# nikolovjovan/exblas

Measured on AMD Instinct MI355X. Metric: ExSUM fp64 Gelem/s at n=2^28 (bit-exact vs CPU superaccumulator/MPFR), higher is better.
Workload: dtype f64; 1 GPU; ExSUM n=2^28 fp64 ill_cond(c=1e+32), fpe=8 early_exit=True, 1xMI355X, inputs resident in HBM, steps rotate over 4 distinct vectors; n_total=268435456, fpe=8, early_exit=True, parallelism=single

## Files before the change

exblas_amd/csrc/blas1.hip:

```cpp
#include "superacc.hip.h"
#include "fpe.hip.h"
#include "exblas_internal.h"
#include <hip/hip_ext.h>

namespace exb {

constexpr int BLOCK = 256;
constexpr int WAVES = BLOCK / 64;
constexpr int U = 4;

template <int N, bool EE, int COPIES, int CNT, int ZM = 0>
__device__ __forceinline__ void fpe_absorb(double (&a)[N > 0 ? N : 1], double (&x)[CNT], int from,
                                           long long *col, unsigned &flags)
{
    LdsSink<COPIES> sink{col, flags};
    fpe_absorb_sink<N, EE, CNT, LdsSink<COPIES>, ZM>(a, x, from, sink);
}

template <int N, int COPIES>
__device__ __forceinline__ void fpe_flush(double (&a)[N > 0 ? N : 1], long long *col, unsigned &flags)
{
    LdsSink<COPIES> sink{col, flags};
    fpe_flush_sink<N>(a, sink);
}

template <int COPIES>
__device__ __forceinline__ void block_epilogue(long long *s_acc, unsigned flags, long long *gacc,
                                               unsigned *gflags, int ngroups)
{
    __shared__ unsigned s_flags;
    if (threadIdx.x == 0) s_flags = 0;
    __syncthreads();
    if (flags) atomicOr(&s_flags, flags);
    long long *g = gacc + (size_t)(blockIdx.x % ngroups) * NL;
    for (int l = threadIdx.x; l < NL; l += BLOCK) {
        long long sum = 0;
#pragma unroll
        for (int w = 0; w < WAVES; ++w)
#pragma unroll
            for (int c = 0; c < COPIES; ++c) sum += s_acc[(w * NL + l) * COPIES + c];
        if (sum != 0) atomicAdd((unsigned long long *)&g[l], (unsigned long long)sum);
    }
    __syncthreads();
    if (threadIdx.x == 0 && s_flags) atomicOr(gflags, s_flags);
}

template <int N, bool EE, int COPIES>
__global__ void __launch_bounds__(BLOCK) k_exsum(const double *__restrict__ a, long long n,
                                                 long long *__restrict__ gacc,
                                                 unsigned *__restrict__ gflags, int ngroups)
{
    __shared__ long long s_acc[WAVES * NL * COPIES];
    auto zero_lds = [&]() {
        for (int i = threadIdx.x; i < WAVES * NL * COPIES; i += BLOCK) s_acc[i] = 0;
        __syncthreads();
    };
    const int wave = threadIdx.x >> 6, lane = threadIdx.x & 63;
    long long *col = s_acc + wave * NL * COPIES + (lane & (COPIES - 1));
    unsigned flags = 0;
    double fpe[N > 0 ? N : 1];
#pragma unroll
    for (int i = 0; i < (N > 0 ? N : 1); ++i) fpe[i] = 0.0;

    const long long head = (((uintptr_t)a & 8u) && n > 0) ? 1 : 0;
    const d2_t *v = (const d2_t *)(a + head);
    const long long nv = (n - head) >> 1;
    constexpr long long TILE = (long long)BLOCK * U;
    const long long ntiles = nv / TILE;
    LdsSink<COPIES> sinkm{col, flags};
    Bypass bypass;

    long long t = blockIdx.x;
    if (t < ntiles) {
        d2_t r0[U], r1[U];
        auto fill = [&](long long tile, d2_t (&r)[U]) {
            const d2_t *p = v + (tile < ntiles ? tile : ntiles - 1) * TILE + threadIdx.x;
#pragma unroll
            for (int u = 0; u < U; ++u) r[u] = ld2(p + u * BLOCK);
        };
        auto absorb = [&](d2_t (&r)[U]) {
            double x[2 * U];
#pragma unroll
            for (int u = 0; u < U; ++u) {
                x[2 * u] = r[u].x;
                x[2 * u + 1] = r[u].y;
            }
            fpe_absorb_adaptive<N, EE, 2 * U, LdsSink<COPIES>>(fpe, x, sinkm, bypass);
        };
        fill(t, r0);
        zero_lds();
        for (;;) {
            fill(t + gridDim.x, r1);
            absorb(r0);
            t += gridDim.x;
            if (t >= ntiles) break;
            fill(t + gridDim.x, r0);
            absorb(r1);
            t += gridDim.x;
            if (t >= ntiles) break;
        }
    } else {
        zero_lds();
    }
    for (long long i = ntiles * TILE + (long long)blockIdx.x * BLOCK + threadIdx.x; i < nv;
         i += (long long)gridDim.x * BLOCK) {
        d2_t r = v[i];
        double x[2] = {r.x, r.y};
        fpe_absorb<N, false, COPIES, 2>(fpe, x, 0, col, flags);
    }
    if (blockIdx.x == 0 && threadIdx.x == 0) {
        if (head) lds_add<COPIES>(col, a[0], flags);
        if ((n - head) & 1) lds_add<COPIES>(col, a[n - 1], flags);
    }
    fpe_flush<N, COPIES>(fpe, col, flags);
    block_epilogue<COPIES>(s_acc, flags, gacc, gflags, ngroups);
}

template <int N, bool EE, int COPIES>
__global__ void __launch_bounds__(BLOCK) k_exsum_strided(const double *__restrict__ a, long long n,
                                                         long long inca, long long *__restrict__ gacc,
                                                         unsigned *__restrict__ gflags, int ngroups)
{
    __shared__ long long s_acc[WAVES * NL * COPIES];
    for (int i = threadIdx.x; i < WAVES * NL * COPIES; i += BLOCK) s_acc[i] = 0;
    __syncthreads();
    const int wave = threadIdx.x >> 6, lane = threadIdx.x & 63;
    long long *col = s_acc + wave * NL * COPIES + (lane & (COPIES - 1));
    unsigned flags = 0;
    double fpe[N > 0 ? N : 1];
#pragma unroll
    for (int i = 0; i < (N > 0 ? N : 1); ++i) fpe[i] = 0.0;
    const long long T = (long long)gridDim.x * BLOCK;
    for (long long i = (long long)blockIdx.x * BLOCK + threadIdx.x; i < n; i += 4 * T) {
        double x[4];
#pragma unroll
        for (int u = 0; u < 4; ++u) x[u] = i + u * T < n ? a[(i + u * T) * inca] : 0.0;
        fpe_absorb<N, false, COPIES, 4>(fpe, x, 0, col, flags);
    }
    fpe_flush<N, COPIES>(fpe, col, flags);
    block_epilogue<COPIES>(s_acc, flags, gacc, gflags, ngroups);
}

template <int N, bool EE, int COPIES, int ZM>
__global__ void __launch_bounds__(BLOCK) k_exdot(const double *__restrict__ a, const double *__restrict__ b,
                                                 long long n, long long *__restrict__ gacc,
                                                 unsigned *__restrict__ gflags, int ngroups)
{
    __shared__ long long s_acc[WAVES * NL * COPIES];
    auto zero_lds = [&]() {
        for (int i = threadIdx.x; i < WAVES * NL * COPIES; i += BLOCK) s_acc[i] = 0;
        __syncthreads();
    };
    const int wave = threadIdx.x >> 6, lane = threadIdx.x & 63;
    long long *col = s_acc + wave * NL * COPIES + (lane & (COPIES - 1));
    unsigned flags = 0;
    LdsSink<COPIES> sink{col, flags};
    long long *const lo_acc = low_acc_of(gflags), *const hi_acc = high_acc_of(gflags);
    double fpe[N > 0 ? N : 1];
#pragma unroll
    for (int i = 0; i < (N > 0 ? N : 1); ++i) fpe[i] = 0.0;

    const d2_t *va = (const d2_t *)a, *vb = (const d2_t *)b;
    const long long nv = n >> 1;
    Bypass bypass;
    constexpr long long TILE = (long long)BLOCK * U;
    const long long ntiles = nv / TILE;
    long long t = blockIdx.x;
    d2_t ra[U], rb[U];
    if (t < ntiles) {
        const long long base = t * TILE + threadIdx.x;
#pragma unroll
        for (int u = 0; u < U; ++u) {
            ra[u] = ld2(va + base + u * BLOCK);
            rb[u] = ld2(vb + base + u * BLOCK);
        }
    }
    zero_lds();
    if (t < ntiles) {
        d2_t rc[U], rd[U];
        auto fill = [&](long long tile, d2_t (&pa)[U], d2_t (&pb)[U]) {
            const long long base = (tile < ntiles ? tile : ntiles - 1) * TILE + threadIdx.x;
#pragma unroll
            for (int u = 0; u < U; ++u) {
                pa[u] = ld2(va + base + u * BLOCK);
                pb[u] = ld2(vb + base + u * BLOCK);
            }
        };
        auto absorb = [&](d2_t (&pa)[U], d2_t (&pb)[U]) {
            double x[2 * U], e[2 * U];
#pragma unroll
            for (int u = 0; u < U; ++u) {
                x[2 * u] = two_prod(pa[u].x, pb[u].x, e[2 * u]);
                x[2 * u + 1] = two_prod(pa[u].y, pb[u].y, e[2 * u + 1]);
            }
            if (!prod_range_divert<2 * U>(fpe[0], x, e, sink, lo_acc, hi_acc, [&](int j) { return j & 1 ? pa[j >> 1].y : pa[j >> 1].x; },
                                              [&](int j) { return j & 1 ? pb[j >> 1].y : pb[j >> 1].x; }))
                fpe_absorb_prod_adaptive<N, EE, 2 * U, LdsSink<COPIES>, ZM, false>(fpe, x, e, sink, bypass);
        };
        for (;;) {
            fill(t + gridDim.x, rc, rd);
            absorb(ra, rb);
            t += gridDim.x;
            if (t >= ntiles) break;
            fill(t + gridDim.x, ra, rb);
            absorb(rc, rd);
            t += gridDim.x;
            if (t >= ntiles) break;
        }
    }
    for (long long i = ntiles * TILE + (long long)blockIdx.x * BLOCK + threadIdx.x; i < nv;
         i += (long long)gridDim.x * BLOCK) {
        d2_t ra = va[i], rb = vb[i];
        double x[2], e[2];
        x[0] = two_prod(ra.x, rb.x, e[0]);
        x[1] = two_prod(ra.y, rb.y, e[1]);
        if (!prod_range_divert<2>(fpe[0], x, e, sink, lo_acc, hi_acc, [&](int j) { return j ? ra.y : ra.x; }, [&](int j) { return j ? rb.y : rb.x; }))
            fpe_absorb_prod<N, false, 2, LdsSink<COPIES>, 0, false>(fpe, x, e, sink);
    }
    if (blockIdx.x == 0 && threadIdx.x == 0 && (n & 1)) {
        double x1[1], e1[1];
        x1[0] = two_prod(a[n - 1], b[n - 1], e1[0]);
        if (!prod_range_divert<1>(fpe[0], x1, e1, sink, lo_acc, hi_acc, [&](int) { return a[n - 1]; }, [&](int) { return b[n - 1]; }))
            sink_product(sink, x1[0], e1[0]);
    }
    fpe_flush<N, COPIES>(fpe, col, flags);
    block_epilogue<COPIES>(s_acc, flags, gacc, gflags, ngroups);
}

template <int N, bool EE, int COPIES>
__global__ void __launch_bounds__(BLOCK) k_exdot_strided(const double *__restrict__ a, long long inca,
                                                         const double *__restrict__ b, long long incb,
                                                         long long n, long long *__restrict__ gacc,
                                                         unsigned *__restrict__ gflags, int ngroups)
{
    __shared__ long long s_acc[WAVES * NL * COPIES];
    for (int i = threadIdx.x; i < WAVES * NL * COPIES; i += BLOCK) s_acc[i] = 0;
    __syncthreads();
    const int wave = threadIdx.x >> 6, lane = threadIdx.x & 63;
    long long *col = s_acc + wave * NL * COPIES + (lane & (COPIES - 1));
    unsigned flags = 0;
    LdsSink<COPIES> sink{col, flags};
    long long *const lo_acc = low_acc_of(gflags), *const hi_acc = high_acc_of(gflags);
    double fpe[N > 0 ? N : 1];
#pragma unroll
    for (int i = 0; i < (N > 0 ? N : 1); ++i) fpe[i] = 0.0;
    const long long T = (long long)gridDim.x * BLOCK;
    for (long long i = (long long)blockIdx.x * BLOCK + threadIdx.x; i < n; i += 4 * T) {
        double va[4], vb[4], x[4], e[4];
#pragma unroll
        for (int u = 0; u < 4; ++u) {
            const bool in = i + u * T < n;
            va[u] = in ? a[(i + u * T) * inca] : 0.0;
            vb[u] = in ? b[(i + u * T) * incb] : 0.0;
        }
#pragma unroll
        for (int u = 0; u < 4; ++u) x[u] = two_prod(va[u], vb[u], e[u]);
        if (!prod_range_divert<4>(fpe[0], x, e, sink, lo_acc, hi_acc, [&](int j) { return va[j]; }, [&](int j) { return vb[j]; }))
            fpe_absorb_prod<N, false, 4, LdsSink<COPIES>, 0, false>(fpe, x, e, sink);
    }
    fpe_flush<N, COPIES>(fpe, col, flags);
    block_epilogue<COPIES>(s_acc, flags, gacc, gflags, ngroups);
}

__global__ void __launch_bounds__(64) k_finalize(long long *sets, int nsets, int set_stride, unsigned *gflags,
                                                 unsigned flags_or, int zero_sets, long long *out,
                                                 const long long *ext_in, long long *ext_out)
{
    const int lane = threadIdx.x;
    unsigned flags = flags_or;
    if (gflags) flags |= *gflags;
    if (set_stride >= SET_WORDS) {
        for (int g = 0; g < nsets; ++g)
        {
            for (int k = 0; k < 3; ++k)
                if (sets[(size_t)g * set_stride + NL + k] != 0) flags |= (1u << k);
            const long long pw = sets[(size_t)g * set_stride + NL + 3];
            if (pw & 0xffff) flags |= FLAG_PUNDER;
            if (pw >> 16) flags |= FLAG_POVER;
        }
    }
    long long lo0 = 0, hi0 = 0, lo1 = 0, hi1 = 0;
    for (int g0 = 0; g0 < nsets; g0 += 16) {
        long long t0[16], t1[16];
#pragma unroll
        for (int k = 0; k < 16; ++k) {
            const bool ok = g0 + k < nsets;
            const long long *p = sets + (size_t)(ok ? g0 + k : 0) * set_stride;
            t0[k] = ok ? __builtin_nontemporal_load(p + lane) : 0;
            t1[k] = (ok && lane < NL - 64) ? __builtin_nontemporal_load(p + 64 + lane) : 0;
        }
#pragma unroll
        for (int k = 0; k < 16; ++k) {
            lo0 += t0[k] & 0xffffffffll;
            hi0 += t0[k] >> 32;
            if (lane == NL - 65) {
                lo1 += t1[k];
            } else {
                lo1 += t1[k] & 0xffffffffll;
                hi1 += t1[k] >> 32;
            }
        }
    }
    long long in0 = __shfl_up(hi0, 1), in1 = __shfl_up(hi1, 1);
    const long long h63 = __shfl(hi0, 63);
    if (lane == 0) { in0 = 0; in1 = h63; }
    long long v0 = lo0 + in0, v1 = (lane < NL - 64) ? lo1 + in1 : 0;
    if (zero_sets) {
        for (int i = lane; i < nsets * set_stride; i += 64) sets[i] = 0;
        if (lane == 0 && gflags) *gflags = 0;
    }
    __shared__ long long s_v[NL], s_lo[NL], s_hi[NL], s_c[NL + EXT_SHIFT_DIGITS];
    __shared__ unsigned long long s_ex;
    __shared__ int s_over;
    bool low_folded = false;
    const bool have_low = (flags & FLAG_PUNDER) && (ext_in || gflags);
    const bool have_high = (flags & FLAG_POVER) && (ext_in || gflags);
    if (ext_out) {
        if (!have_low) {
            ext_out[lane] = 0;
            if (lane < SET_WORDS - 64) ext_out[64 + lane] = 0;
        }
        if (!have_high) {
            ext_out[SET_WORDS + lane] = 0;
            if (lane < SET_WORDS - 64) ext_out[SET_WORDS + 64 + lane] = 0;
        }
    }
    if (have_low || have_high) {
        const long long *lsrc = ext_in ? ext_in : low_acc_of(gflags);
        const long long *hsrc = ext_in ? ext_in + SET_WORDS : high_acc_of(gflags);
        s_lo[lane] = have_low ? lsrc[lane] : 0;
        s_hi[lane] = have_high ? hsrc[lane] : 0;
        s_v[lane] = v0;
        if (lane < NL - 64) {
            s_lo[64 + lane] = have_low ? lsrc[64 + lane] : 0;
            s_hi[64 + lane] = have_high ? hsrc[64 + lane] : 0;
            s_v[64 + lane] = v1;
        }
        if (!ext_in && zero_sets) {
            long long *lo = low_acc_of(gflags), *hi = high_acc_of(gflags);
            if (have_low) {
                lo[lane] = 0;
                if (lane < NL - 64) lo[64 + lane] = 0;
            }
            if (have_high) {
                hi[lane] = 0;
                if (lane < NL - 64) hi[64 + lane] = 0;
            }
        }
        __syncthreads();
        if (lane == 0) {
            s_over = 0;
            if (have_low) normalize_digits(s_lo);
            if (have_high) normalize_digits(s_hi);
            if (!ext_out) {
                if (have_high) s_over = fold_high_digits(s_v, s_hi, s_c);
                if (have_low && !s_over) {
                    for (int j = LOW_SHIFT_DIGITS; j < NL; ++j) s_v[j - LOW_SHIFT_DIGITS] += s_lo[j];
                    normalize_digits(s_v);
                    const bool half = (s_lo[LOW_SHIFT_DIGITS - 1] >> 31) & 1ll;
                    bool sticky = (s_lo[LOW_SHIFT_DIGITS - 1] & 0x7fffffffll) != 0;
                    for (int j = 0; j < LOW_SHIFT_DIGITS - 1; ++j) sticky = sticky || s_lo[j] != 0;
                    s_ex = round_exact_bits_frac(s_v, half, sticky);
                }
            }
        }
        __syncthreads();
        if (ext_out) {
            if (have_low) {
                ext_out[lane] = s_lo[lane];
                if (lane < SET_WORDS - 64) ext_out[64 + lane] = lane < NL - 64 ? s_lo[64 + lane] : 0;
            }
            if (have_high) {
                ext_out[SET_WORDS + lane] = s_hi[lane];
                if (lane < SET_WORDS - 64) ext_out[SET_WORDS + 64 + lane] = lane < NL - 64 ? s_hi[64 + lane] : 0;
            }
        } else {
            const int over = s_over;
            if (over) {
                flags |= over > 0 ? FLAG_PINF : FLAG_NINF;
            } else {
                v0 = s_v[lane];
                v1 = lane < NL - 64 ? s_v[64 + lane] : 0;
                low_folded = have_low;
            }
            if (have_low) flags |= FLAG_PLOW_EXACT;
            if (have_high) flags |= FLAG_PHIGH_EXACT;
        }
    }
    WaveFinish r = finish_wave(v0, v1, flags);
    if (low_folded && !(flags & FLAG_NONFINITE)) r.ex = s_ex;
    write_record_wave(r, flags, out);
}

template <int N, bool EE>
__global__ void __launch_bounds__(BLOCK) k_exsum_segmented(const double *__restrict__ values,
                                                           const long long *__restrict__ offsets, long long nseg,
                                                           int round_mode, double *__restrict__ out)
{
    __shared__ long long acc[WAVES][NL];
    __shared__ unsigned fl[WAVES];
    const int lane = threadIdx.x & 63, w = threadIdx.x >> 6;
    const long long seg = (long long)blockIdx.x * WAVES + w;
    const bool valid = seg < nseg;
    for (int t = lane; t < NL; t += 64) acc[w][t] = 0;
    if (lane == 0) fl[w] = 0;
    __syncthreads();
    if (valid) {
        unsigned flags = 0;
        LdsSink<1> sink{acc[w], flags};
        double fpe[N > 0 ? N : 1];
#pragma unroll
        for (int i = 0; i < (N > 0 ? N : 1); ++i) fpe[i] = 0.0;
        const long long b = offsets[seg], e = offsets[seg + 1];
        for (long long i0 = b; i0 < e; i0 += 64) {
            const long long i = i0 + lane;
            double x[1] = {i < e ? values[i] : 0.0};
            fpe_absorb_sink<N, EE, 1>(fpe, x, 0, sink);
        }
        fpe_flush_sink<N>(fpe, sink);
        if (flags) atomicOr(&fl[w], flags);
    }
    __syncthreads();
    const WaveFinish r = finish_wave(acc[w][lane], lane < NL - 64 ? acc[w][64 + lane] : 0, fl[w]);
    if (valid && lane == 0) out[seg] = round_mode ? r.rf : __longlong_as_double((long long)r.ex);
}


#define EXB_LAUNCH_STREAMING(c, kernel, grid, st, ...)                                                                \
    do {                                                                                                               \
        if ((c).launch_stop_event || (c).launch_start_event) {                                                         \
            hipEvent_t ev0_ = (c).launch_start_event, ev1_ = (c).launch_stop_event;                                    \
            (c).launch_start_event = (c).launch_stop_event = nullptr;                                                  \
            hipExtLaunchKernelGGL(kernel, dim3(grid), dim3(BLOCK), 0, st, ev0_, ev1_, 0, __VA_ARGS__);                 \
        } else {                                                                                                       \
            hipLaunchKernelGGL(kernel, dim3(grid), dim3(BLOCK), 0, st, __VA_ARGS__);                                   \
        }                                                                                                              \
    } while (0)

static inline int grid_for(const Ctx &c, long long work_items, long long per_block, int blocks_per_cu)
{
    long long want = (work_items + per_block - 1) / per_block;
    long long cap = (long long)c.num_cu * blocks_per_cu;
    if (want < 1) want = 1;
    if (want >= cap) return (int)max(1ll, cap + c.grid_adj);
    return (int)want;
}

template <int N, bool EE, int COPIES>
static void run_exsum(Ctx &c, const double *a, long long n, hipStream_t st)
{
    const int bpc = N == 0 ? c.bpc_sa : ((!SKIP_ZERO_LEVELS<EE> && N >= 5) ? c.bpc_heavy : c.bpc_sum);
    int grid = grid_for(c, n, (long long)BLOCK * 2 * U, bpc);
    if (grid == c.num_cu * bpc && grid > 1 && !(grid & 1)) grid -= 1;
    EXB_LAUNCH_STREAMING(c, (k_exsum<N, EE, COPIES>), grid, st, a, n, c.gacc, c.gflags, c.ngroups);
}

#ifndef EXBLAS_SUM_COPIES
#define EXBLAS_SUM_COPIES 8
#endif
#ifndef EXBLAS_DOT_COPIES
#define EXBLAS_DOT_COPIES 8
#endif
template <int N, bool EE>
static hipError_t launch_exsum(Ctx &c, const double *a, long long n, long long inca, hipStream_t st)
{
    constexpr int COPIES = (N == 0) ? 16 : EXBLAS_SUM_COPIES;
    if (inca == 1) {
        run_exsum<N, EE, COPIES>(c, a, n, st);
    } else {
        int grid = grid_for(c, n, BLOCK, c.blocks_per_cu);
        EXB_LAUNCH_STREAMING(c, (k_exsum_strided<N, EE, COPIES>), grid, st, a, n, inca, c.gacc, c.gflags, c.ngroups);
    }
    return hipGetLastError();
}

template <int N, bool EE, int COPIES>
static void run_exdot(Ctx &c, const double *a, const double *b, long long n, hipStream_t st)
{
    const long long tiles = n / ((long long)BLOCK * 2 * U);
    const int bpc = (int)min((long long)c.bpc_dot, max(4ll, tiles / (5ll * c.num_cu)));
    int grid = grid_for(c, n, (long long)BLOCK * 2 * U, bpc);
    if (grid > c.num_cu && !(grid & 1)) grid += 1;
    EXB_LAUNCH_STREAMING(c, (k_exdot<N, EE, COPIES, SKIP_ZERO_LEVELS<EE> ? 1 : 0>), grid, st, a, b, n, c.gacc, c.gflags,
                         c.ngroups);
}

template <int N, bool EE>
static hipError_t launch_exdot(Ctx &c, const double *a, long long inca, const double *b, long long incb,
                               long long n, hipStream_t st)
{
    constexpr int COPIES = (N == 0) ? 16 : EXBLAS_DOT_COPIES;
    const bool vec = inca == 1 && incb == 1 && (((uintptr_t)a | (uintptr_t)b) & 15u) == 0;
    if (vec) {
        run_exdot<N, EE, COPIES>(c, a, b, n, st);
    } else {
        int grid = grid_for(c, n, BLOCK, c.blocks_per_cu);
        EXB_LAUNCH_STREAMING(c, (k_exdot_strided<N, EE, COPIES>), grid, st, a, inca, b, incb, n, c.gacc, c.gflags,
                             c.ngroups);
    }
    return hipGetLastError();
}

hipError_t finalize_groups(Ctx &c, hipStream_t st, long long *d_out, long long *d_ext_out)
{
    hipLaunchKernelGGL(k_finalize, dim3(1), dim3(64), 0, st, c.gacc, c.ngroups, NL, c.gflags, 0u, 1, d_out,
                       (const long long *)nullptr, d_ext_out);
    return hipGetLastError();
}

hipError_t finalize_sets(const long long *d_sets, int nsets, unsigned flags_or, hipStream_t st, long long *d_out,
                         const long long *d_ext_sets)
{
    hipLaunchKernelGGL(k_finalize, dim3(1), dim3(64), 0, st, const_cast<long long *>(d_sets), nsets, SET_WORDS,
                       (unsigned *)nullptr, flags_or, 0, d_out, d_ext_sets, (long long *)nullptr);
    return hipGetLastError();
}

hipError_t exsum_dispatch(Ctx &c, const double *a, long long n, long long inca, int fpe, int early_exit,
                          hipStream_t st, bool *supported)
{
    *supported = true;
    if (fpe < 2) return launch_exsum<0, false>(c, a, n, inca, st);
    if (early_exit) {
        if (fpe <= 4) return launch_exsum<4, true>(c, a, n, inca, st);
        if (fpe <= 6) return launch_exsum<6, true>(c, a, n, inca, st);
        if (fpe <= 8) return launch_exsum<8, true>(c, a, n, inca, st);
    } else {
        switch (fpe) {
        case 2: return launch_exsum<2, false>(c, a, n, inca, st);
        case 3: return launch_exsum<3, false>(c, a, n, inca, st);
        case 4: return launch_exsum<4, false>(c, a, n, inca, st);
        case 5: return launch_exsum<5, false>(c, a, n, inca, st);
        case 6: return launch_exsum<6, false>(c, a, n, inca, st);
        case 7: return launch_exsum<7, false>(c, a, n, inca, st);
        default: return launch_exsum<8, false>(c, a, n, inca, st);
        }
    }
    *supported = false;
    return hipSuccess;
}

hipError_t exsum_segmented_dispatch(const double *values, const long long *offsets, long long nseg, int fpe,
                                    int early_exit, int round_mode, hipStream_t st, double *out)
{
    if (nseg <= 0) return hipSuccess;
    const dim3 grid((unsigned)((nseg + WAVES - 1) / WAVES)), block(BLOCK);
#define SEG_GO(N, EE) \
    hipLaunchKernelGGL((k_exsum_segmented<N, EE>), grid, block, 0, st, values, offsets, nseg, round_mode, out)
    if (fpe < 2) SEG_GO(0, false);
    else if (early_exit) {
        if (fpe <= 4) SEG_GO(4, true);
        else if (fpe <= 6) SEG_GO(6, true);
        else if (fpe <= 8) SEG_GO(8, true);
        else return hipMemsetAsync(out, 0, sizeof(double) * nseg, st);
    } else {
        switch (fpe) {
        case 2: SEG_GO(2, false); break;
        case 3: SEG_GO(3, false); break;
        case 4: SEG_GO(4, false); break;
        case 5: SEG_GO(5, false); break;
        case 6: SEG_GO(6, false); break;
        case 7: SEG_GO(7, false); break;
        default: SEG_GO(8, false); break;
        }
    }
#undef SEG_GO
    return hipGetLastError();
}

hipError_t exdot_dispatch(Ctx &c, const double *a, long long inca, const double *b, long long incb, long long n,
                          int fpe, int early_exit, hipStream_t st, bool *supported)
{
    *supported = true;
    if (fpe < 3) return launch_exdot<0, false>(c, a, inca, b, incb, n, st);
    if (early_exit) {
        if (fpe <= 4) return launch_exdot<4, true>(c, a, inca, b, incb, n, st);
        if (fpe <= 6) return launch_exdot<6, true>(c, a, inca, b, incb, n, st);
        if (fpe <= 8) return launch_exdot<8, true>(c, a, inca, b, incb, n, st);
    } else {
        switch (fpe) {
        case 3: return launch_exdot<3, false>(c, a, inca, b, incb, n, st);
        case 4: return launch_exdot<4, false>(c, a, inca, b, incb, n, st);
        case 5: return launch_exdot<5, false>(c, a, inca, b, incb, n, st);
        case 6: return launch_exdot<6, false>(c, a, inca, b, incb, n, st);
        case 7: return launch_exdot<7, false>(c, a, inca, b, incb, n, st);
        default: return launch_exdot<8, false>(c, a, inca, b, incb, n, st);
        }
    }
    *supported = false;
    return hipSuccess;
}

}
```

exblas_amd/csrc/fpe.hip.h:

```cpp
#pragma once
#include "superacc.hip.h"

namespace exb {

typedef double d2_t __attribute__((ext_vector_type(2)));

__device__ __forceinline__ d2_t ld2(const d2_t *p) { return __builtin_nontemporal_load(p); }

__device__ __forceinline__ unsigned expo_field(double x) { return ((unsigned)__double2hiint(x) >> 20) & 0x7ffu; }
constexpr unsigned BIG_EXPO = 1023u + 1000u;
constexpr unsigned LOW_EXPO = 1023u - 968u;

template <int CNT, int ZM = 0>
__device__ __forceinline__ bool any_nonzero(const double (&x)[CNT])
{
    if constexpr (ZM == 0) {
        unsigned bits = 0;
#pragma unroll
        for (int j = 0; j < CNT; ++j)
            bits |= ((unsigned)__double2hiint(x[j]) << 1) | (unsigned)__double2loint(x[j]);
        return bits != 0;
    } else {
        bool nz = false;
#pragma unroll
        for (int j = 0; j < CNT; ++j) nz |= (x[j] != 0.0);
        return nz;
    }
}

template <int COPIES>
struct LdsSink {
    long long *col;
    unsigned &flags;
    __device__ __forceinline__ void add(double x) { lds_add<COPIES>(col, x, flags); }
    __device__ __forceinline__ void note(unsigned bits) { flags |= bits; }
};

struct GlobalSink {
    long long *acc;
    __device__ __forceinline__ void note(unsigned) {}
    __device__ __forceinline__ void add(double x)
    {
        const unsigned long long u = (unsigned long long)__double_as_longlong(x);
        unsigned be = (unsigned)(u >> 52) & 0x7ffu;
        unsigned long long m = u & 0x000fffffffffffffull;
        if (be == 0x7ffu) {
            atomicAdd((unsigned long long *)&acc[NL + (m ? 2 : ((u >> 63) ? 1 : 0))], 1ull);
            return;
        }
        if (be) m |= 0x0010000000000000ull; else be = 1u;
        const unsigned p = be - 1u;
        const unsigned idx = p >> 5, sh = p & 31u;
        const unsigned long long lo = m << sh;
        const unsigned hi = (unsigned)((m >> 32) >> (32u - sh));
        long long c0 = (long long)(lo & 0xffffffffull), c1 = (long long)(lo >> 32), c2 = (long long)hi;
        if (u >> 63) { c0 = -c0; c1 = -c1; c2 = -c2; }
        unsigned long long *q = (unsigned long long *)(acc + idx);
        if (c0) atomicAdd(q, (unsigned long long)c0);
        if (c1) atomicAdd(q + 1, (unsigned long long)c1);
        if (c2) atomicAdd(q + 2, (unsigned long long)c2);
    }
};

template <class Sink>
__device__ __forceinline__ void sink_product(Sink &sink, double p, double e)
{
    sink.add(p);
    if (expo_field(p) != 0x7ffu) {
        if (e != 0.0) sink.add(e);
    } else if (__builtin_isinf(p) && __builtin_isinf(e)) {
        sink.note(FLAG_POVER);
    }
}

template <int CNT, class Sink, class FA, class FB>
__device__ __forceinline__ bool prod_range_divert(double &a0, const double (&p)[CNT], const double (&e)[CNT], Sink &sink,
                                                  long long *lo, long long *hi, FA &&a_of, FB &&b_of)
{
    unsigned mn = 0x7ffu, mx = expo_field(a0);
#pragma unroll
    for (int j = 0; j < CNT; ++j) {
        const unsigned ex = expo_field(p[j]);
        mn = min(mn, ex);
        mx = max(mx, ex);
    }
    if (__builtin_expect(!__any(mn < LOW_EXPO || mx >= BIG_EXPO), 1)) return false;
    bool hz = mx >= BIG_EXPO;
#pragma unroll
    for (int j = 0; j < CNT; ++j) hz |= expo_field(p[j]) < LOW_EXPO && a_of(j) != 0.0 && b_of(j) != 0.0;
    if (!__any(hz)) return false;
    GlobalSink low{lo}, high{hi};
#pragma unroll
    for (int j = 0; j < CNT; ++j) {
        const double a = a_of(j), b = b_of(j);
        const unsigned ex = expo_field(p[j]);
        if (ex < LOW_EXPO && a != 0.0 && b != 0.0) {
            int ea;
            const double a1 = frexp(a, &ea);
            const double b1 = ldexp(b, EXT_SHIFT_BITS + ea);
            const double P = a1 * b1, E = __builtin_fma(a1, b1, -P);
            low.add(P);
            if (E != 0.0) low.add(E);
            sink.note(FLAG_PUNDER);
        } else if (ex == 0x7ffu && expo_field(a) != 0x7ffu && expo_field(b) != 0x7ffu) {
            int ea;
            const double a1 = frexp(a, &ea);
            const double b1 = ldexp(b, ea - EXT_SHIFT_BITS);
            const double P = a1 * b1, E = __builtin_fma(a1, b1, -P);
            high.add(P);
            if (E != 0.0) high.add(E);
            sink.note(FLAG_POVER);
        } else {
            sink_product(sink, p[j], e[j]);
        }
    }
    if (expo_field(a0) >= BIG_EXPO) {
        sink.add(a0);
        a0 = 0.0;
    }
    return true;
}

template <int CNT, class Sink>
__device__ __forceinline__ bool fpe_guard(double &a0, const double (&x)[CNT], const double *e, Sink &sink)
{
    unsigned mx = expo_field(a0);
#pragma unroll
    for (int j = 0; j < CNT; ++j) mx = max(mx, expo_field(x[j]));
    if (__builtin_expect(!__any(mx >= BIG_EXPO), 1)) return false;
#pragma unroll
    for (int j = 0; j < CNT; ++j) {
        if (e) sink_product(sink, x[j], e[j]);
        else sink.add(x[j]);
    }
    if (expo_field(a0) >= BIG_EXPO) {
        sink.add(a0);
        a0 = 0.0;
    }
    return true;
}

#ifndef EXBLAS_FULL_CASCADE
#define EXBLAS_FULL_CASCADE 0
#endif
template <bool EE>
inline constexpr bool SKIP_ZERO_LEVELS = EE || !EXBLAS_FULL_CASCADE;

template <int N, bool EE, int CNT, class Sink, int ZM = 0>
__device__ __forceinline__ bool fpe_cascade(double (&a)[N > 0 ? N : 1], double (&x)[CNT], int from, Sink &sink)
{
    bool live = true;
#pragma unroll
    for (int i = 0; i < N; ++i) {
        if (i >= from && live) {
#pragma unroll
            for (int j = 0; j < CNT; ++j) {
                double s;
                a[i] = two_sum(a[i], x[j], s);
                x[j] = s;
            }
            if (SKIP_ZERO_LEVELS<EE> && i > from) live = __any(any_nonzero<CNT, ZM>(x));
        }
    }
    const bool spill = live && __any(any_nonzero<CNT, ZM>(x));
    if (spill) {
#pragma unroll
        for (int j = 0; j < CNT; ++j)
            if (x[j] != 0.0) sink.add(x[j]);
    }
    return spill;
}

template <int N, bool EE, int CNT, class Sink, int ZM = 0>
__device__ __forceinline__ bool fpe_absorb_sink(double (&a)[N > 0 ? N : 1], double (&x)[CNT], int from, Sink &sink)
{
    if constexpr (N == 0) {
#pragma unroll
        for (int j = 0; j < CNT; ++j) sink.add(x[j]);
        return false;
    } else {
        if (from == 0 && fpe_guard<CNT>(a[0], x, nullptr, sink)) return true;
        return fpe_cascade<N, EE, CNT, Sink, ZM>(a, x, from, sink);
    }
}

#ifndef EXBLAS_BYPASS_MIN
#define EXBLAS_BYPASS_MIN 63
#define EXBLAS_BYPASS_MAX 4095
#endif
constexpr int BYPASS_MIN = EXBLAS_BYPASS_MIN, BYPASS_MAX = EXBLAS_BYPASS_MAX;

struct Bypass {
    int left = 0;
    int span = BYPASS_MIN;
    __device__ __forceinline__ void spilled()
    {
        left = span;
        span = min(2 * span + 1, BYPASS_MAX);
    }
};

template <int N, bool EE, int CNT, class Sink, int ZM = 0>
__device__ __forceinline__ void fpe_absorb_adaptive(double (&a)[N > 0 ? N : 1], double (&x)[CNT], Sink &sink, Bypass &bp)
{
    if constexpr (N == 0) {
        fpe_absorb_sink<N, EE, CNT, Sink, ZM>(a, x, 0, sink);
    } else {
        if (__builtin_expect(bp.left > 0, 0)) {
            --bp.left;
#pragma unroll
            for (int j = 0; j < CNT; ++j) sink.add(x[j]);
        } else if (fpe_absorb_sink<N, EE, CNT, Sink, ZM>(a, x, 0, sink)) {
            bp.spilled();
        } else {
            bp.span = BYPASS_MIN;
        }
    }
}

template <int N, bool EE, int CNT, class Sink, int ZM = 0, bool GUARD = true>
__device__ __forceinline__ bool fpe_absorb_prod(double (&a)[N > 0 ? N : 1], double (&p)[CNT], double (&e)[CNT],
                                                Sink &sink)
{
    if constexpr (N == 0) {
#pragma unroll
        for (int j = 0; j < CNT; ++j) {
            sink_product(sink, p[j], e[j]);
        }
        return false;
    } else {
        constexpr int EFROM = (N >= 3) ? N - 3 : 0;
        if constexpr (GUARD) {
            if (fpe_guard<CNT>(a[0], p, e, sink)) return true;
        }
        const bool s1 = fpe_cascade<N, EE, CNT, Sink, ZM>(a, p, 0, sink);
        const bool s2 = fpe_cascade<N, EE, CNT, Sink, ZM>(a, e, EFROM, sink);
        return s1 || s2;
    }
}

template <int N, bool EE, int CNT, class Sink, int ZM = 0, bool GUARD = true>
__device__ __forceinline__ void fpe_absorb_prod_adaptive(double (&a)[N > 0 ? N : 1], double (&p)[CNT],
                                                         double (&e)[CNT], Sink &sink, Bypass &bp)
{
    if constexpr (N == 0) {
        fpe_absorb_prod<N, EE, CNT>(a, p, e, sink);
    } else {
        if (__builtin_expect(bp.left > 0, 0)) {
            --bp.left;
#pragma unroll
            for (int j = 0; j < CNT; ++j) {
                sink_product(sink, p[j], e[j]);
            }
        } else if (fpe_absorb_prod<N, EE, CNT, Sink, ZM, GUARD>(a, p, e, sink)) {
            bp.spilled();
        } else {
            bp.span = BYPASS_MIN;
        }
    }
}

template <int N, class Sink>
__device__ __forceinline__ void fpe_flush_sink(double (&a)[N > 0 ? N : 1], Sink &sink)
{
    if constexpr (N > 0) {
#pragma unroll
        for (int i = 0; i < N; ++i) {
            if (a[i] != 0.0) sink.add(a[i]);
            a[i] = 0.0;
        }
    }
}

}
```

exblas_amd/csrc/superacc.hip.h:

```cpp
#pragma once
#include <hip/hip_runtime.h>
#include <stdint.h>

namespace exb {

constexpr int NL = 68;
constexpr int CANON = 41;
constexpr int CANON_DIGITS = 52;
constexpr int CANON_FWORDS = 21;

constexpr int OUT_EXACT = 0;
constexpr int OUT_REFMODE = 1;
constexpr int OUT_FLAGS = 2;
constexpr int OUT_CANON = 4;
constexpr int OUT_DIGITS = 48;
constexpr int OUT_FLAGCNT = 116;
constexpr int SET_WORDS = 72;
constexpr int OUT_WORDS = 128;

constexpr unsigned FLAG_PINF = 1u, FLAG_NINF = 2u, FLAG_NAN = 4u;
constexpr unsigned FLAG_PUNDER = 8u, FLAG_POVER = 16u, FLAG_NONFINITE = 7u;
constexpr unsigned FLAG_PLOW_EXACT = 32u, FLAG_PHIGH_EXACT = 64u;
constexpr int EXT_SHIFT_DIGITS = 38, EXT_SHIFT_BITS = 32 * EXT_SHIFT_DIGITS;
constexpr int LOW_SHIFT_DIGITS = EXT_SHIFT_DIGITS, LOW_SHIFT_BITS = EXT_SHIFT_BITS;
constexpr int EXT_WORDS = 2 * SET_WORDS;
constexpr int FLAG_BLOCK_BYTES = 64 + EXT_WORDS * 8;
__device__ __forceinline__ long long *low_acc_of(unsigned *gflags) { return (long long *)((char *)gflags + 64); }
__device__ __forceinline__ long long *high_acc_of(unsigned *gflags) { return low_acc_of(gflags) + SET_WORDS; }

__device__ __forceinline__ double two_sum(double a, double b, double &s)
{
    double r = a + b;
    double z = r - a;
    s = (a - (r - z)) + (b - z);
    return r;
}

__device__ __forceinline__ double two_prod(double a, double b, double &e)
{
    double p = a * b;
    e = __builtin_fma(a, b, -p);
    return p;
}

__device__ __forceinline__ double two_prod_safe(double a, double b, double &e)
{
    double p = a * b;
    double t = __builtin_fma(a, b, -p);
    e = __builtin_isfinite(p) ? t : 0.0;
    return p;
}

template <int COPIES>
__device__ __forceinline__ void lds_add(long long *col, double x, unsigned &flags)
{
    const unsigned long long u = (unsigned long long)__double_as_longlong(x);
    unsigned be = (unsigned)(u >> 52) & 0x7ffu;
    unsigned long long m = u & 0x000fffffffffffffull;
    if (be == 0x7ffu) {
        flags |= m ? FLAG_NAN : ((u >> 63) ? FLAG_NINF : FLAG_PINF);
        return;
    }
    if (be) m |= 0x0010000000000000ull; else be = 1u;
    const unsigned p = be - 1u;
    const unsigned idx = p >> 5, sh = p & 31u;
    const unsigned long long lo = m << sh;
    const unsigned hi = (unsigned)((m >> 32) >> (32u - sh));
    long long c0 = (long long)(lo & 0xffffffffull);
    long long c1 = (long long)(lo >> 32);
    long long c2 = (long long)hi;
    if (u >> 63) { c0 = -c0; c1 = -c1; c2 = -c2; }
    unsigned long long *q = (unsigned long long *)(col + idx * COPIES);
    atomicAdd(q, (unsigned long long)c0);
    atomicAdd(q + COPIES, (unsigned long long)c1);
    atomicAdd(q + 2 * COPIES, (unsigned long long)c2);
}

__device__ inline void normalize_digits(long long *v, int nd = NL)
{
    long long carry = 0;
    for (int i = 0; i < nd - 1; ++i) {
        long long t = v[i] + carry;
        carry = t >> 32;
        v[i] = t & 0xffffffffll;
    }
    v[nd - 1] += carry;
}

__device__ inline int fold_high_digits(long long *v, const long long *h, long long *c)
{
    constexpr int ND = NL + EXT_SHIFT_DIGITS;
    for (int i = 0; i < ND; ++i) c[i] = (i < NL ? v[i] : 0) + (i >= EXT_SHIFT_DIGITS ? h[i - EXT_SHIFT_DIGITS] : 0);
    normalize_digits(c, ND);
    bool zeros = c[ND - 1] == 0, ones = c[ND - 1] == -1;
    for (int i = NL; i < ND - 1; ++i) {
        zeros = zeros && c[i] == 0;
        ones = ones && c[i] == 0xffffffffll;
    }
    if (ones && !((c[NL - 1] >> 31) & 1)) ones = false;
    if (zeros && ((c[NL - 1] >> 31) & 1)) zeros = false;
    if (!zeros && !ones) return c[ND - 1] < 0 ? -1 : 1;
    for (int i = 0; i < NL - 1; ++i) v[i] = c[i];
    v[NL - 1] = zeros ? c[NL - 1] : c[NL - 1] - 0x100000000ll;
    return 0;
}

__device__ inline unsigned long long round_exact_bits(const long long *v)
{
    const bool neg = v[NL - 1] < 0;
    unsigned mag[NL];
    if (!neg) {
        for (int i = 0; i < NL; ++i) mag[i] = (unsigned)v[i];
    } else {
        unsigned long long c = 1;
        for (int i = 0; i < NL; ++i) {
            unsigned long long t = (unsigned long long)(~(unsigned)v[i]) + c;
            mag[i] = (unsigned)t;
            c = t >> 32;
        }
    }
    int t = NL - 1;
    while (t >= 0 && mag[t] == 0) --t;
    const unsigned long long sign = neg ? 0x8000000000000000ull : 0ull;
    if (t < 0) return 0ull;
    const int lz = __builtin_clz(mag[t]);
    const int msb = 32 * t + 31 - lz;
    if (msb <= 52) {
        unsigned long long val = ((unsigned long long)(t >= 1 ? mag[1] : 0u) << 32) | mag[0];
        return sign | val;
    }
    const unsigned d1 = (t >= 1) ? mag[t - 1] : 0u, d2 = (t >= 2) ? mag[t - 2] : 0u;
    unsigned long long w = ((unsigned long long)mag[t] << 32) | d1;
    unsigned rest;
    if (lz) {
        w = (w << lz) | (unsigned long long)(d2 >> (32 - lz));
        rest = d2 << lz;
    } else {
        rest = d2;
    }
    bool sticky = (w & 0x3ffull) != 0 || rest != 0;
    for (int i = t - 3; i >= 0 && !sticky; --i) sticky = mag[i] != 0;
    unsigned long long bits = ((unsigned long long)(msb - 52) << 52) + (w >> 11);
    const bool rnd = (w >> 10) & 1ull;
    if (rnd && (sticky || (bits & 1ull))) bits += 1;
    if ((bits >> 52) >= 0x7ffull) bits = 0x7ff0000000000000ull;
    return sign | bits;
}

__device__ inline unsigned long long round_exact_bits_frac(const long long *v, bool half, bool sticky)
{
    if (!half && !sticky) return round_exact_bits(v);
    const bool neg = v[NL - 1] < 0;
    unsigned mag[NL];
    if (!neg) {
        for (int i = 0; i < NL; ++i) mag[i] = (unsigned)v[i];
    } else {
        for (int i = 0; i < NL; ++i) mag[i] = ~(unsigned)v[i];
        const bool h = half, st = sticky;
        half = !(h && st);
        sticky = !(h && !st);
    }
    const unsigned long long sign = neg ? 0x8000000000000000ull : 0ull;
    int t = NL - 1;
    while (t >= 0 && mag[t] == 0) --t;
    const int lz = t >= 0 ? __builtin_clz(mag[t]) : 0;
    const int msb = t >= 0 ? 32 * t + 31 - lz : -1;
    if (msb <= 52) {
        unsigned long long val = t < 0 ? 0ull : (((unsigned long long)(t >= 1 ? mag[1] : 0u) << 32) | mag[0]);
        if (half && (sticky || (val & 1ull))) val += 1;
        return sign | val;
    }
    const unsigned d1 = (t >= 1) ? mag[t - 1] : 0u, d2 = (t >= 2) ? mag[t - 2] : 0u;
    unsigned long long w = ((unsigned long long)mag[t] << 32) | d1;
    unsigned rest;
    if (lz) {
        w = (w << lz) | (unsigned long long)(d2 >> (32 - lz));
        rest = d2 << lz;
    } else {
        rest = d2;
    }
    bool st2 = true;
    (void)rest;
    unsigned long long bits = ((unsigned long long)(msb - 52) << 52) + (w >> 11);
    const bool rnd = (w >> 10) & 1ull;
    if (rnd && (st2 || (bits & 1ull))) bits += 1;
    if ((bits >> 52) >= 0x7ffull) bits = 0x7ff0000000000000ull;
    return sign | bits;
}

__device__ inline long long digits_field52(const long long *v, int o)
{
    const int q = o >> 5, r = o & 31;
    auto dig = [&](int i) -> unsigned long long {
        if (i < 0) return 0ull;
        if (i >= NL - 1) {
            const long long top = v[NL - 1];
            const int k = i - (NL - 1);
            if (k == 0) return (unsigned long long)(unsigned)top;
            if (k == 1) return (unsigned long long)(unsigned)(top >> 32);
            return (top < 0) ? 0xffffffffull : 0ull;
        }
        return (unsigned long long)(unsigned)v[i];
    };
    const unsigned long long lo = dig(q) | (dig(q + 1) << 32);
    const unsigned long long hi = dig(q + 2) | (dig(q + 3) << 32);
    const unsigned long long win = r ? ((lo >> r) | (hi << (64 - r))) : lo;
    return (long long)(win & ((1ull << CANON_DIGITS) - 1));
}

__device__ inline void digits_to_canon(const long long *v, long long *canon)
{
    for (int j = 0; j < CANON - 1; ++j) canon[j] = digits_field52(v, CANON_DIGITS * j - 18);
    const int o = CANON_DIGITS * (CANON - 1) - 18;
    const int q = o >> 5, r = o & 31;
    auto dig = [&](int i) -> unsigned long long {
        if (i >= NL - 1) {
            const long long top = v[NL - 1];
            const int k = i - (NL - 1);
            if (k == 0) return (unsigned long long)(unsigned)top;
            if (k == 1) return (unsigned long long)(unsigned)(top >> 32);
            return (top < 0) ? 0xffffffffull : 0ull;
        }
        return (unsigned long long)(unsigned)v[i];
    };
    const unsigned long long lo = dig(q) | (dig(q + 1) << 32);
    const unsigned long long hi = dig(q + 2) | (dig(q + 3) << 32);
    canon[CANON - 1] = (long long)(r ? ((lo >> r) | (hi << (64 - r))) : lo);
}

__device__ inline double round_reference(const long long *acc)
{
    const long long mask = (1ll << CANON_DIGITS) - 1;
    const bool negative = acc[CANON - 1] < 0;
    int i;
    for (i = CANON - 1; i >= 0 && acc[i] == 0; --i) { }
    if (negative) {
        for (; i >= 0 && (acc[i] & mask) == mask; --i) { }
    }
    if (i < 0) return 0.0;
    long long hiword = negative ? mask - acc[i] : acc[i];
    double rounded = (double)hiword;
    double hi = ldexp(rounded, (i - CANON_FWORDS) * CANON_DIGITS);
    if (i == 0) return negative ? -hi : hi;
    hiword -= __double2ll_rn(rounded);
    double mid = ldexp((double)hiword, (i - CANON_FWORDS) * CANON_DIGITS);
    long long sticky = 0;
    for (int j = 0; j != i - 1; ++j) sticky |= negative ? (1ll << CANON_DIGITS) - acc[j] : acc[j];
    long long loword = negative ? (1ll << CANON_DIGITS) - acc[i - 1] : acc[i - 1];
    loword |= (sticky != 0);
    double lo = ldexp((double)loword, (i - 1 - CANON_FWORDS) * CANON_DIGITS);
    if (mid != 0) {
        unsigned long long b = (unsigned long long)__double_as_longlong(mid + lo);
        b |= (unsigned long long)(lo != 0.0);
        lo = __longlong_as_double((long long)b);
    }
    hi = hi + lo;
    return negative ? -hi : hi;
}

__device__ inline void finish_record(long long *v, unsigned flags, long long *out)
{
    normalize_digits(v);
    long long canon[CANON];
    digits_to_canon(v, canon);
    unsigned long long ex = round_exact_bits(v);
    double rf = round_reference(canon);
    if (flags & FLAG_NONFINITE) {
        const bool nan = (flags & FLAG_NAN) || ((flags & FLAG_PINF) && (flags & FLAG_NINF));
        ex = nan ? 0x7ff8000000000000ull
                 : ((flags & FLAG_NINF) ? 0xfff0000000000000ull : 0x7ff0000000000000ull);
        rf = __longlong_as_double((long long)ex);
    }
    out[OUT_EXACT] = (long long)ex;
    out[OUT_REFMODE] = __double_as_longlong(rf);
    out[OUT_FLAGS] = (long long)flags;
    out[3] = 0;
    for (int j = 0; j < CANON; ++j) out[OUT_CANON + j] = canon[j];
    for (int j = 0; j < NL; ++j) out[OUT_DIGITS + j] = v[j];
    out[OUT_FLAGCNT + 0] = (flags & FLAG_PINF) ? 1 : 0;
    out[OUT_FLAGCNT + 1] = (flags & FLAG_NINF) ? 1 : 0;
    out[OUT_FLAGCNT + 2] = (flags & FLAG_NAN) ? 1 : 0;
    out[OUT_FLAGCNT + 3] = ((flags & FLAG_PUNDER) ? 1 : 0) + ((flags & FLAG_POVER) ? 65536 : 0);
}

__device__ __forceinline__ long long wave_shr1(long long v)
{
    int lo = (int)v, hi = (int)(v >> 32);
    lo = __builtin_amdgcn_update_dpp(0, lo, 0x138, 0xf, 0xf, true);
    hi = __builtin_amdgcn_update_dpp(0, hi, 0x138, 0xf, 0xf, true);
    return (long long)(((unsigned long long)(unsigned)hi << 32) | (unsigned long long)(unsigned)lo);
}
__device__ __forceinline__ unsigned lane_bcast(unsigned v, int l)
{
    return (unsigned)__builtin_amdgcn_readlane((int)v, l);
}
__device__ __forceinline__ long long lane_bcast(long long v, int l)
{
    const unsigned lo = lane_bcast((unsigned)v, l), hi = lane_bcast((unsigned)(v >> 32), l);
    return (long long)(((unsigned long long)hi << 32) | lo);
}
__device__ __forceinline__ double lane_bcast(double v, int l)
{
    return __longlong_as_double(lane_bcast(__double_as_longlong(v), l));
}

__device__ __forceinline__ void wave_add_double(long long &v0, long long &v1, double x, unsigned &flags)
{
    const int lane = (int)(threadIdx.x & 63u);
    const unsigned long long u = (unsigned long long)__double_as_longlong(x);
    unsigned be = (unsigned)(u >> 52) & 0x7ffu;
    unsigned long long m = u & 0x000fffffffffffffull;
    if (be == 0x7ffu) {
        flags |= m ? FLAG_NAN : ((u >> 63) ? FLAG_NINF : FLAG_PINF);
        return;
    }
    if (be) m |= 0x0010000000000000ull; else be = 1u;
    const unsigned p = be - 1u;
    const int idx = (int)(p >> 5);
    const unsigned sh = p & 31u;
    const unsigned long long lo = m << sh;
    const unsigned hi = (unsigned)((m >> 32) >> (32u - sh));
    long long c0 = (long long)(lo & 0xffffffffull), c1 = (long long)(lo >> 32), c2 = (long long)hi;
    if (u >> 63) { c0 = -c0; c1 = -c1; c2 = -c2; }
    const int k0 = lane - idx;
    const int k1 = lane + 64 - idx;
    v0 += k0 == 0 ? c0 : (k0 == 1 ? c1 : (k0 == 2 ? c2 : 0ll));
    if (lane < NL - 64) v1 += k1 == 0 ? c0 : (k1 == 1 ? c1 : (k1 == 2 ? c2 : 0ll));
}

struct WaveFinish {
    unsigned long long ex;
    double rf;
    long long canon;
    long long d0, d1;
};

template <bool FULL = true>
__device__ inline WaveFinish finish_wave(long long v0, long long v1, const unsigned flags)
{
    const int lane = (int)(threadIdx.x & 63u);
    constexpr int HI = NL - 64;
    if (lane >= HI) v1 = 0;
    const unsigned long long nzA = __ballot(v0 != 0), nzB = __ballot(v1 != 0);
    const int hi = nzB ? 64 + (63 - __builtin_clzll(nzB)) : (nzA ? 63 - __builtin_clzll(nzA) : -1);
    const bool split0 = lane <= hi;
    const bool split1 = (64 + lane <= hi) && (lane < HI - 1);
    for (int pass = 0; pass < 2 * NL && hi >= 0; ++pass) {
        const long long c0 = split0 ? (v0 >> 32) : 0, lo0 = split0 ? (v0 & 0xffffffffll) : v0;
        const long long c1 = split1 ? (v1 >> 32) : 0, lo1 = split1 ? (v1 & 0xffffffffll) : v1;
        long long in0 = wave_shr1(c0), in1 = wave_shr1(c1);
        const long long c63 = lane_bcast(c0, 63);
        if (lane == 0) in1 = c63;
        v0 = lo0 + in0;
        v1 = (lane < HI) ? lo1 + in1 : 0;
        const bool pending = (split0 && (v0 >> 32) != 0) || (split1 && (v1 >> 32) != 0);
        if (!__any(pending)) break;
    }
    if (hi >= 0 && hi + 1 < NL - 1) {
        const int e = hi + 1;
        const long long s0 = lane_bcast(v0, e & 63), s1 = lane_bcast(v1, (e - 64) & 63);
        const long long sv = e < 64 ? s0 : s1;
        const long long fill = sv < 0 ? 0xffffffffll : 0ll;
        if (lane == e) v0 = sv & 0xffffffffll;
        if (lane > e) v0 = fill;
        if (lane < HI) {
            const int i1 = 64 + lane;
            if (i1 == e) v1 = sv & 0xffffffffll;
            if (i1 > e) v1 = (i1 == NL - 1) ? (sv < 0 ? -1ll : 0ll) : fill;
        }
    }
    WaveFinish r;
    r.d0 = v0;
    r.d1 = v1;
    const long long top = lane_bcast(v1, HI - 1);
    const bool neg = top < 0;
    const unsigned d0 = (unsigned)v0, d1 = (unsigned)v1;
    const unsigned long long nz0 = __ballot(d0 != 0), nz1 = __ballot(lane < HI && d1 != 0);
    const int z = nz0 ? __builtin_ctzll(nz0) : (nz1 ? 64 + __builtin_ctzll(nz1) : NL);
    const int i1 = 64 + lane;
    const unsigned m0 = !neg ? d0 : (lane < z ? 0u : (lane == z ? (0u - d0) : ~d0));
    const unsigned m1 = (lane >= HI) ? 0u : (!neg ? d1 : (i1 < z ? 0u : (i1 == z ? (0u - d1) : ~d1)));
    const unsigned long long mz0 = __ballot(m0 != 0), mz1 = __ballot(m1 != 0);
    const int tp = mz1 ? 64 + (63 - __builtin_clzll(mz1)) : (mz0 ? 63 - __builtin_clzll(mz0) : -1);
    auto mag = [&](int i) -> unsigned {
        const unsigned a = lane_bcast(m0, i & 63), b = lane_bcast(m1, (i - 64) & 63);
        return i < 0 ? 0u : (i < 64 ? a : b);
    };
    unsigned long long ex = 0ull;
    const unsigned long long sign = neg ? 0x8000000000000000ull : 0ull;
    {
        const unsigned mt = mag(tp < 0 ? 0 : tp), ma = mag(tp - 1), mb = mag(tp - 2), q0 = mag(0), q1 = mag(1);
        if (tp >= 0) {
            const int lz = __builtin_clz(mt | 1u);
            const int msb = 32 * tp + 31 - lz;
            if (msb <= 52) {
                ex = sign | (((unsigned long long)(tp >= 1 ? q1 : 0u) << 32) | q0);
            } else {
                unsigned long long w = ((unsigned long long)mt << 32) | ma;
                unsigned rest = mb;
                if (lz) {
                    w = (w << lz) | (unsigned long long)(mb >> (32 - lz));
                    rest = mb << lz;
                }
                const bool sticky = (w & 0x3ffull) != 0 || rest != 0 || z < tp - 2;
                unsigned long long bits = ((unsigned long long)(msb - 52) << 52) + (w >> 11);
                if (((w >> 10) & 1ull) && (sticky || (bits & 1ull))) bits += 1;
                if ((bits >> 52) >= 0x7ffull) bits = 0x7ff0000000000000ull;
                ex = sign | bits;
            }
        }
    }
    double rf = 0.0;
    r.canon = 0;
    if constexpr (FULL) {
    auto digit = [&](int i) -> unsigned long long {
        const unsigned a = __shfl(d0, i & 63), b = __shfl(d1, (i - 64) & 63);
        const int k = i - (NL - 1);
        unsigned v = (i < 64) ? a : b;
        if (k == 0) v = (unsigned)top;
        if (k == 1) v = (unsigned)(top >> 32);
        if (k >= 2) v = neg ? 0xffffffffu : 0u;
        return i < 0 ? 0ull : (unsigned long long)v;
    };
    {
        const int j = lane < CANON ? lane : 0;
        const int o = CANON_DIGITS * j - 18;
        const int q = o >> 5, sh = o & 31;
        const unsigned long long lo = digit(q) | (digit(q + 1) << 32), hi = digit(q + 2) | (digit(q + 3) << 32);
        const unsigned long long win = sh ? ((lo >> sh) | (hi << (64 - sh))) : lo;
        r.canon = (j == CANON - 1) ? (long long)win : (long long)(win & ((1ull << CANON_DIGITS) - 1));
    }
    {
        const long long mask = (1ll << CANON_DIGITS) - 1;
        const long long cj = r.canon;
        const bool in = lane < CANON;
        const unsigned long long lead = __ballot(in && (neg ? ((cj & mask) != mask) : (cj != 0)));
        const unsigned long long nzc = __ballot(in && cj != 0);
        const int i = lead ? 63 - __builtin_clzll(lead) : -1;
        const int cz = nzc ? __builtin_ctzll(nzc) : CANON;
        const long long ci = __shfl(cj, i < 0 ? 0 : i), cl = __shfl(cj, i < 1 ? 0 : i - 1);
        if (i >= 0) {
            long long hiword = neg ? mask - ci : ci;
            const double rounded = (double)hiword;
            double hi = ldexp(rounded, (i - CANON_FWORDS) * CANON_DIGITS);
            if (i == 0) {
                rf = neg ? -hi : hi;
            } else {
                hiword -= __double2ll_rn(rounded);
                const double mid = ldexp((double)hiword, (i - CANON_FWORDS) * CANON_DIGITS);
                const bool sticky = neg ? (i >= 2) : (cz < i - 1);
                long long loword = neg ? (1ll << CANON_DIGITS) - cl : cl;
                loword |= (long long)sticky;
                double lo = ldexp((double)loword, (i - 1 - CANON_FWORDS) * CANON_DIGITS);
                if (mid != 0) {
                    unsigned long long b = (unsigned long long)__double_as_longlong(mid + lo);
                    b |= (unsigned long long)(lo != 0.0);
                    lo = __longlong_as_double((long long)b);
                }
                hi = hi + lo;
                rf = neg ? -hi : hi;
            }
        }
    }
    }
    if (flags & FLAG_NONFINITE) {
        const bool nan = (flags & FLAG_NAN) || ((flags & FLAG_PINF) && (flags & FLAG_NINF));
        ex = nan ? 0x7ff8000000000000ull : ((flags & FLAG_NINF) ? 0xfff0000000000000ull : 0x7ff0000000000000ull);
        rf = __longlong_as_double((long long)ex);
    }
    r.ex = ex;
    r.rf = rf;
    return r;
}

__device__ inline void write_record_wave(const WaveFinish &r, unsigned flags, long long *out)
{
    const int lane = (int)(threadIdx.x & 63u);
    if (lane == 0) {
        out[OUT_EXACT] = (long long)r.ex;
        out[OUT_REFMODE] = __double_as_longlong(r.rf);
        out[OUT_FLAGS] = (long long)flags;
        out[3] = 0;
        out[OUT_FLAGCNT + 0] = (flags & FLAG_PINF) ? 1 : 0;
        out[OUT_FLAGCNT + 1] = (flags & FLAG_NINF) ? 1 : 0;
        out[OUT_FLAGCNT + 2] = (flags & FLAG_NAN) ? 1 : 0;
        out[OUT_FLAGCNT + 3] = ((flags & FLAG_PUNDER) ? 1 : 0) + ((flags & FLAG_POVER) ? 65536 : 0);
    }
    if (lane < CANON) out[OUT_CANON + lane] = r.canon;
    out[OUT_DIGITS + lane] = r.d0;
    if (lane < NL - 64) out[OUT_DIGITS + 64 + lane] = r.d1;
}

}
```

Baseline: 861.9 Gelem/s.

## Add deep-prefetch direct LDS path for bypass mode with finite-only scatter

When the adaptive bypass is active, the sum loop now enters a dedicated direct path. It keeps up to three tiles of loads in flight across four register buffers and scatters each element straight into the LDS superaccumulator. A new lds_add_finite applies the sign to the mantissa with a branchless negation and skips the NaN/Inf check whenever a wavefront-wide max-exponent test rules out non-finite values. The product path also uses the finite scatter when the guard is disabled. This trades more registers and code size for hiding load latency on ill-conditioned inputs, where the bypass is hit often.

```diff
diff --git a/exblas_amd/csrc/blas1.hip b/exblas_amd/csrc/blas1.hip
--- a/exblas_amd/csrc/blas1.hip
+++ b/exblas_amd/csrc/blas1.hip
@@ -87,13 +87,63 @@
             }
             fpe_absorb_adaptive<N, EE, 2 * U, LdsSink<COPIES>>(fpe, x, sinkm, bypass);
         };
+        auto direct = [&](d2_t (&s0)[U]) {
+            d2_t s1[U] = {}, s2[U] = {}, s3[U] = {};
+            const long long G = gridDim.x;
+            auto load = [&](long long tile, d2_t (&r)[U]) {
+                if (tile < ntiles) {
+                    const d2_t *p = v + tile * TILE + threadIdx.x;
+#pragma unroll
+                    for (int u = 0; u < U; ++u) r[u] = ld2(p + u * BLOCK);
+                }
+            };
+            auto copy = [&](d2_t (&r)[U]) {
+                if (t < ntiles) {
+#pragma unroll
+                    for (int u = 0; u < U; ++u) s0[u] = r[u];
+                }
+            };
+            auto step = [&](d2_t (&cur)[U], d2_t (&far)[U]) -> bool {
+                if (bypass.left >= 3) load(t + 3 * G, far);
+                double x[2 * U];
+#pragma unroll
+                for (int u = 0; u < U; ++u) {
+                    x[2 * u] = cur[u].x;
+                    x[2 * u + 1] = cur[u].y;
+                }
+                direct_tile<2 * U>(x, sinkm);
+                t += G;
+                return --bypass.left == 0 || t >= ntiles;
+            };
+            load(t + G, s1);
+            if (bypass.left >= 2) load(t + 2 * G, s2);
+            for (;;) {
+                if (step(s0, s3)) { copy(s1); break; }
+                if (step(s1, s0)) { copy(s2); break; }
+                if (step(s2, s1)) { copy(s3); break; }
+                if (step(s3, s2)) break;
+            }
+        };
         fill(t, r0);
         zero_lds();
         for (;;) {
+            if constexpr (N > 0) {
+                if (__builtin_expect(bypass.left > 0, 0)) {
+                    direct(r0);
+                    if (t >= ntiles) break;
+                }
+            }
             fill(t + gridDim.x, r1);
             absorb(r0);
             t += gridDim.x;
             if (t >= ntiles) break;
+            if constexpr (N > 0) {
+                if (__builtin_expect(bypass.left > 0, 0)) {
+#pragma unroll
+                    for (int u = 0; u < U; ++u) r0[u] = r1[u];
+                    continue;
+                }
+            }
             fill(t + gridDim.x, r0);
             absorb(r1);
             t += gridDim.x;
diff --git a/exblas_amd/csrc/fpe.hip.h b/exblas_amd/csrc/fpe.hip.h
--- a/exblas_amd/csrc/fpe.hip.h
+++ b/exblas_amd/csrc/fpe.hip.h
@@ -33,6 +33,7 @@
     long long *col;
     unsigned &flags;
     __device__ __forceinline__ void add(double x) { lds_add<COPIES>(col, x, flags); }
+    __device__ __forceinline__ void add_finite(double x) { lds_add_finite<COPIES>(col, x); }
     __device__ __forceinline__ void note(unsigned bits) { flags |= bits; }
 };
 
@@ -218,6 +219,31 @@
     }
 }
 
+template <int CNT, class Sink>
+__device__ __forceinline__ void direct_tile(const double (&x)[CNT], Sink &sink)
+{
+    unsigned mx = 0;
+#pragma unroll
+    for (int j = 0; j < CNT; ++j) mx = max(mx, expo_field(x[j]));
+    if (__builtin_expect(__any(mx == 0x7ffu), 0)) {
+#pragma unroll
+        for (int j = 0; j < CNT; ++j) sink.add(x[j]);
+    } else {
+#pragma unroll
+        for (int j = 0; j < CNT; ++j) sink.add_finite(x[j]);
+    }
+}
+
+template <int CNT, class Sink>
+__device__ __forceinline__ void direct_tile_prod(const double (&p)[CNT], const double (&e)[CNT], Sink &sink)
+{
+#pragma unroll
+    for (int j = 0; j < CNT; ++j) {
+        sink.add_finite(p[j]);
+        sink.add_finite(e[j]);
+    }
+}
+
 template <int N, bool EE, int CNT, class Sink, int ZM = 0, bool GUARD = true>
 __device__ __forceinline__ bool fpe_absorb_prod(double (&a)[N > 0 ? N : 1], double (&p)[CNT], double (&e)[CNT],
                                                 Sink &sink)
@@ -248,9 +274,13 @@
     } else {
         if (__builtin_expect(bp.left > 0, 0)) {
             --bp.left;
-#pragma unroll
-            for (int j = 0; j < CNT; ++j) {
-                sink_product(sink, p[j], e[j]);
+            if constexpr (!GUARD) {
+                direct_tile_prod<CNT>(p, e, sink);
+            } else {
+#pragma unroll
+                for (int j = 0; j < CNT; ++j) {
+                    sink_product(sink, p[j], e[j]);
+                }
             }
         } else if (fpe_absorb_prod<N, EE, CNT, Sink, ZM, GUARD>(a, p, e, sink)) {
             bp.spilled();
diff --git a/exblas_amd/csrc/superacc.hip.h b/exblas_amd/csrc/superacc.hip.h
--- a/exblas_amd/csrc/superacc.hip.h
+++ b/exblas_amd/csrc/superacc.hip.h
@@ -73,6 +73,25 @@
     unsigned long long *q = (unsigned long long *)(col + idx * COPIES);
     atomicAdd(q, (unsigned long long)c0);
     atomicAdd(q + COPIES, (unsigned long long)c1);
+    atomicAdd(q + 2 * COPIES, (unsigned long long)c2);
+}
+
+template <int COPIES>
+__device__ __forceinline__ void lds_add_finite(long long *col, double x)
+{
+    const long long u = __double_as_longlong(x);
+    unsigned be = ((unsigned)__double2hiint(x) >> 20) & 0x7ffu;
+    long long m = u & 0x000fffffffffffffll;
+    if (be) m |= 0x0010000000000000ll; else be = 1u;
+    const long long s = u >> 63;
+    m = (m ^ s) - s;
+    const unsigned p = be - 1u;
+    const unsigned idx = p >> 5, sh = p & 31u;
+    const unsigned long long lo = (unsigned long long)m << sh;
+    const long long c2 = (m >> 32) >> (32u - sh);
+    unsigned long long *q = (unsigned long long *)(col + idx * COPIES);
+    atomicAdd(q, lo & 0xffffffffull);
+    atomicAdd(q + COPIES, lo >> 32);
     atomicAdd(q + 2 * COPIES, (unsigned long long)c2);
 }
 
```

Result: slower. 852.1 Gelem/s (-1.1%).
